# lashhw/rtcuda

Measured on AMD Instinct MI355X. Metric: Msamples/s at 1920x1080, bun_zipper.ply, higher is better.
Workload: dtype f32

## Files before the change

rtcuda_amd/csrc/rt_device.h:

```cpp
#ifndef RT_DEVICE_H
#define RT_DEVICE_H

#include <hip/hip_runtime.h>
#include <stdint.h>

#include "rt_pinned_math.h"

#define RT_DEV __device__ __forceinline__
#ifdef RT_ISA_MARKS
#define RT_MARK(name) __asm__ volatile("; RT_MARK " name)
#else
#define RT_MARK(name)
#endif

namespace rt {

constexpr float kInvPi = 0.31830988618379067153f;
constexpr float kTwoPi = 6.28318530717958647692f;
constexpr int kRrStart = 4;
constexpr float kRrThreshold = 1.f;
constexpr float kFltMax = 3.402823466e+38f;
constexpr float kFltEps = 1.192092896e-07f;

struct V3 {
    float x, y, z;
};
RT_DEV V3 mk(float x, float y, float z) { return V3{x, y, z}; }
RT_DEV V3 neg(V3 a) { return mk(-a.x, -a.y, -a.z); }
RT_DEV V3 add(V3 a, V3 b) { return mk(a.x + b.x, a.y + b.y, a.z + b.z); }
RT_DEV V3 sub(V3 a, V3 b) { return mk(a.x - b.x, a.y - b.y, a.z - b.z); }
RT_DEV V3 mul(V3 a, V3 b) { return mk(a.x * b.x, a.y * b.y, a.z * b.z); }
RT_DEV V3 scale(V3 a, float t) { return mk(a.x * t, a.y * t, a.z * t); }
RT_DEV V3 divf(V3 a, float t) {
    float inv_t = 1.f / t;
    return mk(a.x * inv_t, a.y * inv_t, a.z * inv_t);
}
RT_DEV float dot(V3 a, V3 b) { return a.x * b.x + a.y * b.y + a.z * b.z; }
RT_DEV V3 cross(V3 a, V3 b) {
    return mk(a.y * b.z - a.z * b.y, a.z * b.x - a.x * b.z, a.x * b.y - a.y * b.x);
}
RT_DEV float len2(V3 a) { return a.x * a.x + a.y * a.y + a.z * a.z; }
RT_DEV float len(V3 a) { return sqrtf(a.x * a.x + a.y * a.y + a.z * a.z); }
RT_DEV V3 unit(V3 a) {
    float inv_len = 1.f / len(a);
    return mk(a.x * inv_len, a.y * inv_len, a.z * inv_len);
}
RT_DEV float max3(V3 a) { return fmaxf(fmaxf(a.x, a.y), a.z); }
template <int STEPS = 1>
RT_DEV float rcp_exact_normal(float x) {
    float r = __builtin_amdgcn_rcpf(x);
#pragma unroll
    for (int k = 0; k < STEPS; k++) {
        const float e = fmaf(-x, r, 1.f);
        r = fmaf(e, r, r);
    }
    return r;
}
RT_DEV V3 reflect(V3 v, V3 n) { return sub(v, scale(n, 2.f * dot(v, n))); }
RT_DEV V3 refract4(V3 unit_v, V3 unit_n, float eta_ratio, float cos_theta) {
    V3 v_parallel = scale(add(unit_v, scale(unit_n, cos_theta)), eta_ratio);
    V3 v_perp = scale(unit_n, -sqrtf(1.f - len2(v_parallel)));
    return add(v_parallel, v_perp);
}

struct Rng {
    uint32_t d, v0, v1, v2, v3, v4;
};
RT_DEV uint32_t rng_next(Rng &s) {
    uint32_t t = s.v0 ^ (s.v0 >> 2);
    s.v0 = s.v1;
    s.v1 = s.v2;
    s.v2 = s.v3;
    s.v3 = s.v4;
    s.v4 = (s.v4 ^ (s.v4 << 4)) ^ (t ^ (t << 1));
    s.d += 362437u;
    return s.v4 + s.d;
}
RT_DEV Rng rng_sample_stream(uint32_t seed_lo, uint32_t seed_hi, unsigned long long key) {
    unsigned long long z = (((unsigned long long)seed_hi << 32) | seed_lo) + 0x9E3779B97F4A7C15ull * (key + 1ull);
    z = (z ^ (z >> 30)) * 0xBF58476D1CE4E5B9ull;
    z = (z ^ (z >> 27)) * 0x94D049BB133111EBull;
    z ^= z >> 31;
    const uint32_t s0 = (uint32_t)z ^ 0xaad26b49u, s1 = (uint32_t)(z >> 32) ^ 0xf7dcefddu;
    const uint32_t t0 = 1099087573u * s0, t1 = 2591861531u * s1;
    Rng r;
    r.d = 6615241u + t1 + t0;
    r.v0 = 123456789u + t0;
    r.v1 = 362436069u ^ t0;
    r.v2 = 521288629u + t1;
    r.v3 = 88675123u ^ t1;
    r.v4 = 5783321u + t0;
    return r;
}
RT_DEV float rng_to_uniform(uint32_t draw) { return (float)draw * 2.3283064e-10f + (2.3283064e-10f / 2.0f); }
RT_DEV float rng_uniform(Rng &s) { return rng_to_uniform(rng_next(s)); }

struct Tri {
    V3 p0, e1, e2, n;
};
RT_DEV Tri load_tri(const float4 *__restrict__ tris, int k) {
    const float4 *q = (const float4 *)((const char *)tris + __umul24((unsigned)k, 48u));
    float4 a = q[0];
    float4 b = q[1];
    float4 c = q[2];
    Tri t;
    t.p0 = mk(a.x, a.y, a.z);
    t.e1 = mk(a.w, b.x, b.y);
    t.e2 = mk(b.z, b.w, c.x);
    t.n = mk(c.y, c.z, c.w);
    return t;
}
RT_DEV bool tri_intersect(const Tri &tr, V3 o, V3 d, float tmax, float &t_out, float &u_out, float &v_out) {
    V3 c = sub(tr.p0, o);
    V3 r = cross(d, c);
    float inv_det = 1.f / dot(d, tr.n);
    float u = inv_det * dot(tr.e2, r);
    float v = inv_det * dot(tr.e1, r);
    float t = inv_det * dot(c, tr.n);
    t_out = t;
    u_out = u;
    v_out = v;
    return u >= 0.0f && v >= 0.0f && (u + v) <= 1.0f && 0 < t && t <= tmax;
}
RT_DEV V3 tri_point(const Tri &tr, float u, float v) { return add(sub(tr.p0, scale(tr.e1, u)), scale(tr.e2, v)); }
RT_DEV float tri_area(const Tri &tr) { return 0.5f * len(tr.n); }

RT_DEV V3 offset_ray_origin(V3 p, V3 n) {
    const float int_scale = 256.f;
    const float float_scale = 1.f / 65536.f;
    const float origin = 1.f / 32.f;
    int ox = (int)(int_scale * n.x);
    int oy = (int)(int_scale * n.y);
    int oz = (int)(int_scale * n.z);
    float px = __int_as_float(__float_as_int(p.x) + (p.x < 0 ? -ox : ox));
    float py = __int_as_float(__float_as_int(p.y) + (p.y < 0 ? -oy : oy));
    float pz = __int_as_float(__float_as_int(p.z) + (p.z < 0 ? -oz : oz));
    return mk(fabsf(p.x) < origin ? p.x + float_scale * n.x : px,
              fabsf(p.y) < origin ? p.y + float_scale * n.y : py,
              fabsf(p.z) < origin ? p.z + float_scale * n.z : pz);
}
RT_DEV float power_heuristic(float f_pdf, float g_pdf_float) {
    int g = (int)g_pdf_float;
    float f2 = f_pdf * f_pdf;
    return f2 / (f2 + (float)(g * g));
}
RT_DEV bool same_hemisphere(V3 wo, V3 wi, V3 n) { return dot(wo, n) * dot(wi, n) < 0.f; }
RT_DEV V3 uniform_sample_sphere(Rng &rs) {
    float z = 1 - 2 * rng_uniform(rs);
    float r = sqrtf(1 - z * z);
    float phi = kTwoPi * rng_uniform(rs);
    float x, y;
    rt_sincosf(phi, &y, &x);
    return mk(r * x, r * y, z);
}

struct Material {
    float ax, ay, az;
    float ior;
// ... 79 lines not shown
```

rtcuda_amd/csrc/rt_frame_kernels.inc:

```
#ifndef RT_CHUNK_RELEASE_WAIT
#define RT_CHUNK_RELEASE_WAIT 1
#endif

template <bool LDS_TABLES>
__global__ void __launch_bounds__(kBlock)
RT_K_ADVANCE(DScene sc, DPools p, RT_FRAME_SRC cam, AdvanceParams ap, float *__restrict__ fb, DCounters *__restrict__ ctr,
             DWaveRow *__restrict__ rows, unsigned int *__restrict__ lock_shades) {
    if (ap.lockstep >= 3 && lock_shades[ap.lockstep - 2] == 0u) return;
    __shared__ float s_tab[LDS_TABLES ? kTabDwordsMax : 1];
    const int i = blockIdx.x * blockDim.x + threadIdx.x;
    const bool in_range = i < ap.n;
    SlotState st;
    st.bounces = kDone;
    st.hit_info = -1;
    st.pixel = 0;
    st.gen = 0;
    st.rs = Rng{0, 0, 0, 0, 0, 0};
    st.beta = st.wo = st.isect_p = st.isect_n = mk(0, 0, 0);
    if (in_range) {
        st.bounces = p.bounces(i);
        st.hit_info = p.hit_info(i);
        st.pixel = p.pixel(i);
        st.gen = p.gen(i);
        st.rs = Rng{p.rd(i), p.r0(i), p.r1(i), p.r2(i), p.r3(i), p.r4(i)};
        st.beta = mk(p.br(i), p.bg(i), p.bb(i));
        st.wo = mk(p.dx(i), p.dy(i), p.dz(i));
        st.isect_p = mk(p.hpx(i), p.hpy(i), p.hpz(i));
        st.isect_n = mk(p.hnx(i), p.hny(i), p.hnz(i));
    }
    const float *tab = sc.tables;
    if (LDS_TABLES) {
        for (int k = threadIdx.x; k < sc.tab_dwords; k += kBlock) s_tab[k] = sc.tables[k];
        __syncthreads();
        tab = s_tab;
    }
    if (ap.lockstep && st.bounces == kParked) {
        st.bounces = ap.max_bounces;
        st.hit_info = -1;
    }
    const bool alive = st.bounces != kDone && st.bounces != kParked;
    AdvanceOut out;
    out.did_gen = out.did_shade = out.has_shadow = out.did_emit = out.new_ray = false;
    out.rr_draws = 0;
    if (alive) {
        const int gen_before = st.gen;
        advance_core<false>(sc, tab, cam, ap, ap.slot_lo + i, st, out, fb);
        if (out.new_ray) {
            p.ox(i) = out.ray_o.x;
            p.oy(i) = out.ray_o.y;
            p.oz(i) = out.ray_o.z;
            p.dx(i) = out.ray_d.x;
            p.dy(i) = out.ray_d.y;
            p.dz(i) = out.ray_d.z;
        }
        if (st.gen != gen_before) {
            p.gen(i) = st.gen;
            p.pixel(i) = st.pixel;
        }
        if (out.has_shadow) {
            p.sox(i) = out.s_o.x;
            p.soy(i) = out.s_o.y;
            p.soz(i) = out.s_o.z;
            p.sdx(i) = out.s_d.x;
            p.sdy(i) = out.s_d.y;
            p.sdz(i) = out.s_d.z;
            p.slr(i) = out.s_L.x;
            p.slg(i) = out.s_L.y;
            p.slb(i) = out.s_L.z;
            p.starget(i) = out.s_target;
            p.stmax(i) = out.s_tmax;
        }
        p.br(i) = st.beta.x;
        p.bg(i) = st.beta.y;
        p.bb(i) = st.beta.z;
        p.bounces(i) = st.bounces;
        p.rd(i) = st.rs.d;
        p.r0(i) = st.rs.v0;
        p.r1(i) = st.rs.v1;
        p.r2(i) = st.rs.v2;
        p.r3(i) = st.rs.v3;
        p.r4(i) = st.rs.v4;
    }
    if (in_range && !out.has_shadow) p.stmax(i) = -1.f;

    unsigned long long traced = wave_ballot(out.did_gen || out.did_shade);
    int rr_tot = out.rr_draws;
    if (wave_ballot(out.rr_draws != 0)) {
        for (int off = 32; off > 0; off >>= 1) rr_tot += __shfl_xor(rr_tot, off);
    } else {
        rr_tot = 0;
    }
    unsigned long long v[C_COUNT] = {(unsigned long long)wave_count((out.did_gen)),
                                     (unsigned long long)wave_count((out.did_shade)),
                                     (unsigned long long)__popcll(traced),
                                     (unsigned long long)wave_count((out.has_shadow)),
                                     (unsigned long long)wave_count((out.did_emit)),
                                     0ull,
                                     (unsigned long long)rr_tot,
                                     0ull};
    row_add(rows, v);
    if ((ap.round & ap.batch_mask) == ap.batch_mask && traced != 0 && lane_id() == 0) ctr->last_live_round = ap.round;
    if (ap.lockstep) {
        unsigned long long sm = wave_ballot(out.did_shade);
        if (sm != 0 && lane_id() == 0) atomicAdd(&lock_shades[ap.lockstep - 1], (unsigned)__popcll(sm));
    }
}

template <bool LDS_TABLES, bool WIDE, int MIN_WAVES, bool DRAW_CIDS = false, bool LITERAL = false, bool VERIFY = false>
__global__ void __launch_bounds__(kBlock, MIN_WAVES)
RT_K_PATHS(DScene sc, DPools p, RT_FRAME_SRC cam_arg, AdvanceParams ap_arg, float *__restrict__ fb, DWaveRow *__restrict__ rows,
           int stack_cap, int *overflow, int adv_batch, int debug_no_deposit, unsigned long long *prof, int top_n,
           int prio_period, int rot_wave, int rot_set, int gen_batch, int tri_follow, unsigned int *__restrict__ next_cid,
           unsigned long long *__restrict__ vstat) {
    constexpr bool SPLIT_GEN = MIN_WAVES != 2;
    asm volatile("s_nop 0\n\ts_nop 0");
    extern __shared__ int s_lds[];
    int *stack = s_lds + threadIdx.x;
    float *park = (float *)(s_lds + (stack_cap + 1) * kBlock) + threadIdx.x;
    int *over = overflow + (blockIdx.x * kBlock + threadIdx.x) % kOverStride;
    int *cold = s_lds + (stack_cap + 10) * kBlock + threadIdx.x;
    float *acc = (float *)(s_lds + (stack_cap + 23) * kBlock) + threadIdx.x;
    float *s_tab = (float *)(s_lds + (stack_cap + 26) * kBlock);
    const float *tab = sc.tables;
    const float4 *s_top = (const float4 *)(s_tab + (LDS_TABLES ? ((sc.tab_dwords + 3) & ~3) : 0));
    constexpr bool CHUNKS = RT_PATHS_CHUNKS && SPLIT_GEN && !DRAW_CIDS;
    __shared__ __attribute__((aligned(16))) unsigned s_task[CHUNKS ? 8 : 1];
    __shared__ unsigned s_sem[CHUNKS ? rtchunks::kSemWords : 1];
    const unsigned chunk_g0 = (CHUNKS && top_n > 0) ? (unsigned)top_n & ((1u << rtplan::kChunkHeadShift) - 1u) : 0u;
    const unsigned chunk_head0 = (CHUNKS && top_n > 0) ? (unsigned)top_n >> rtplan::kChunkHeadShift : 0u;
    if (CHUNKS) {
        for (unsigned k = threadIdx.x; k < rtchunks::kSemWords; k += kBlock) s_sem[k] = rtchunks::kSemWordInit;
        if (threadIdx.x == 0) {
            const rtchunks::Multiple m = rtchunks::multiple_of(chunk_g0 ? chunk_g0 : 1u);
            s_task[0] = 0u;
            s_task[1] = chunk_g0;
            s_task[2] = m.inv;
            s_task[3] = m.shift;
            s_task[4] = m.limit;
            s_task[5] = chunk_head0;
        }
    }
    const bool chunk_start = CHUNKS && chunk_g0 && chunk_head0 == 0u;
    if (MIN_WAVES != 2) top_n = 0;
    for (int k = threadIdx.x; k < top_n * 4; k += kBlock) ((float4 *)s_top)[k] = sc.nodes[k];
    if (LDS_TABLES) {
        for (int k = threadIdx.x; k < sc.tab_dwords; k += kBlock) s_tab[k] = sc.tables[k];
        tab = s_tab;
    }
    struct Uniforms {
        RT_FRAME_SRC cam;
        AdvanceParams ap;
    };
    static_assert(sizeof(Uniforms) % 4 == 0, "dword copy");
    Uniforms *s_uni = (Uniforms *)(s_top + 4 * (size_t)top_n);
    {
        Uniforms u;
        u.cam = cam_arg;
        u.ap = ap_arg;
        const int *srcw = (const int *)&u;
        for (int k = threadIdx.x; k < (int)(sizeof(Uniforms) / 4); k += kBlock) ((int *)s_uni)[k] = srcw[k];
    }
    __syncthreads();
    const RT_FRAME_SRC &cam = s_uni->cam;
    const AdvanceParams &ap = s_uni->ap;
    const int ap_n = ap_arg.n, ap_max_bounces = ap_arg.max_bounces, ap_fb_fixed = ap_arg.fb_fixed;
    constexpr bool draw_cids = DRAW_CIDS && SPLIT_GEN;
    int cid_next = 0, cid_end = 0;
    const int lanes_in_grid = (int)(gridDim.x * blockDim.x);
    auto slot_of = [&](int set, unsigned lane_in_wg) {
        return rtchunks::slot_of((unsigned)set, blockIdx.x * blockDim.x + lane_in_wg, (unsigned)lanes_in_grid, (unsigned)rot_wave, (unsigned)rot_set);
    };
    int slot_set = 0;
    int i = slot_of(0, threadIdx.x);
    int bounces = kDone, pixel = 0, gen = 0;
    Rng rs{0, 0, 0, 0, 0, 0};
    V3 beta = mk(0, 0, 0);
    auto load_slot = [&](int k) {
        bounces = p.bounces(k);
        pixel = p.pixel(k);
        gen = p.gen(k);
        rs = Rng{p.rd(k), p.r0(k), p.r1(k), p.r2(k), p.r3(k), p.r4(k)};
        beta = mk(p.br(k), p.bg(k), p.bb(k));
    };
    auto store_slot = [&](int k) {
        p.bounces(k) = bounces;
        p.pixel(k) = pixel;
        p.gen(k) = gen;
        p.hit_info(k) = -1;
        p.stmax(k) = -1.f;
        p.br(k) = beta.x;
        p.bg(k) = beta.y;
        p.bb(k) = beta.z;
        p.rd(k) = rs.d;
        p.r0(k) = rs.v0;
        p.r1(k) = rs.v1;
        p.r2(k) = rs.v2;
        p.r3(k) = rs.v3;
        p.r4(k) = rs.v4;
    };
    auto cold_save = [&]() {
        cold[0 * kBlock] = bounces;
        cold[1 * kBlock] = pixel;
        cold[2 * kBlock] = gen;
        cold[3 * kBlock] = (int)rs.d;
        cold[4 * kBlock] = (int)rs.v0;
        cold[5 * kBlock] = (int)rs.v1;
        cold[6 * kBlock] = (int)rs.v2;
        cold[7 * kBlock] = (int)rs.v3;
        cold[8 * kBlock] = (int)rs.v4;
        cold[9 * kBlock] = __float_as_int(beta.x);
        cold[10 * kBlock] = __float_as_int(beta.y);
        cold[11 * kBlock] = __float_as_int(beta.z);
    };
    auto cold_load = [&]() {
        bounces = cold[0 * kBlock];
        pixel = cold[1 * kBlock];
        gen = cold[2 * kBlock];
        rs = Rng{(uint32_t)cold[3 * kBlock], (uint32_t)cold[4 * kBlock], (uint32_t)cold[5 * kBlock],
                 (uint32_t)cold[6 * kBlock], (uint32_t)cold[7 * kBlock], (uint32_t)cold[8 * kBlock]};
        beta = mk(__int_as_float(cold[9 * kBlock]), __int_as_float(cold[10 * kBlock]), __int_as_float(cold[11 * kBlock]));
    };
    int phase = PH_IDLE;
// ... 23 lines not shown
    acc[0 * kBlock] = acc[1 * kBlock] = acc[2 * kBlock] = 0.f;
    if (chunk_start) {
        i = ap_n;
        phase = PH_GEN;
        cold[12 * kBlock] = -1;
    } else if (i < ap_n) {
        load_slot(i);
        phase = (bounces != kDone && bounces != kParked) ? (SPLIT_GEN ? PH_GEN : PH_ADV) : PH_IDLE;
        cold_save();
        cold[12 * kBlock] = -1;
    }
    unsigned long long n_gen = 0, n_shade = 0, n_traced = 0, n_shadow = 0, n_emit = 0, n_deposit = 0, n_rr = 0;
    unsigned n_bg_lane = 0;
#ifdef RT_TRACE_PROFILE
    unsigned long long pf[16] = {0, 0, 0, 0, 0, 0, 0, 0, 0, 0, 0, 0, 0, 0, 0, 0};
    unsigned long long pf_gen_cycles = 0, pf_fin_cycles = 0, pf_fin_lanes = 0, pf_fin_iters = 0;
    unsigned long long pf_handovers = 0, pf_handover_blocks = 0;
    const unsigned long long pf_t0 = __builtin_readcyclecounter();
    unsigned long long pf_last_work = 0;
#endif

    unsigned prio_tick = 0;
    const unsigned prio_rank = (4u * blockIdx.x) / gridDim.x;
    while (true) {
        RT_MARK("loop.head");
        if (prio_period && (prio_tick++ & ((1u << prio_period) - 1u)) == 0u) {
            unsigned lvl = ((prio_tick >> prio_period) + prio_rank) & 3u;
            lvl = max(lvl, prio_rank >> 1);
            switch (lvl) {
                case 0: __builtin_amdgcn_s_setprio(0); break;
                case 1: __builtin_amdgcn_s_setprio(1); break;
                case 2: __builtin_amdgcn_s_setprio(2); break;
                default: __builtin_amdgcn_s_setprio(3); break;
            }
        }
        bool trav = phase == PH_ANY || phase == PH_CLOSEST;
        bool want_node = trav && cur >= 0;
        bool want_tri = trav && ((cur != kEntryDone && cur < 0) || (kSpeculate && pend != kEntryDone));
        int n_adv = wave_count((phase == PH_ADV));
        const int n_genw = wave_count((phase == PH_GEN));
        int n_node = wave_count((want_node));
        int n_tri = wave_count((want_tri));
        if (n_adv + n_genw + n_node + n_tri == 0) break;
        auto retake = [&]() {
            trav = phase == PH_ANY || phase == PH_CLOSEST;
            want_node = trav && cur >= 0;
            want_tri = trav && ((cur != kEntryDone && cur < 0) || (kSpeculate && pend != kEntryDone));
            n_adv = wave_count((phase == PH_ADV));
            n_node = wave_count((want_node));
            n_tri = wave_count((want_tri));
        };
        const bool run_adv = n_adv > 0 && ((n_adv >= adv_batch && 2 * n_adv >= n_node && 2 * n_adv >= n_tri) || n_node + n_tri == 0);
        if (SPLIT_GEN && !run_adv && n_genw > 0 && (n_genw >= gen_batch || n_node + n_tri == 0)) {
            RT_MARK("gen.begin");
#ifdef RT_TRACE_PROFILE
            pf[12]++; pf[15] += n_genw;
            const unsigned long long pf_tg = __builtin_readcyclecounter();
#endif
            AdvanceOut out;
            out.did_gen = out.new_ray = false;
            out.ray_o = o;
            out.ray_d = d;
            bool hand_back = false;
            long long my_cid = -1;
            if (draw_cids) {
                const unsigned long long m = wave_ballot(phase == PH_GEN);
                const int need = (int)__popcll(m), rank = (int)prefix_popc(m);
                int served = 0;
                while (served < need) {
                    if (cid_next == cid_end) {
                        unsigned base = 0;
                        if (lane_id() == 0) base = atomicAdd(next_cid, (unsigned)kCidChunk);
                        static_assert(0x7ffff000u + (unsigned)kCidChunk < 0x7fffffffu, "cid_end must not overflow int");
                        cid_next = (int)min(__builtin_amdgcn_readfirstlane(base), 0x7ffff000u);
                        cid_end = cid_next + kCidChunk;
                    }
                    const int take = min(need - served, cid_end - cid_next);
                    if (phase == PH_GEN && rank >= served && rank < served + take) my_cid = cid_next + (rank - served);
                    cid_next += take;
                    served += take;
                }
            }
            const unsigned chunk_g = CHUNKS ? __builtin_amdgcn_readfirstlane(s_task[1]) : 0u;
            const bool chunk_was_gen = CHUNKS && phase == PH_GEN;
            const int chunk_acc_pixel = CHUNKS ? cold[1 * kBlock] : 0;
            if (CHUNKS && chunk_g) {
                const rtchunks::Multiple chunk_m{s_task[2], s_task[3], s_task[4]};
                const unsigned chunk_head = __builtin_amdgcn_readfirstlane(s_task[5]);
                bool need = phase == PH_GEN && i >= ap_n;
                const bool at_end = phase == PH_GEN && i < ap_n && slot_set >= (int)chunk_head &&
                                    rtchunks::chunk_ends((unsigned)cold[2 * kBlock], chunk_m, cold[0 * kBlock] == kChunkFresh);
                if (wave_ballot(need || at_end)) {
#ifdef RT_TRACE_PROFILE
                    bool pf_released = false;
#endif
                    if (at_end) {
                        cold_load();
                        const bool ends = gen == ap.last_gen || (long long)gen * kW + (ap.slot_lo + i) >= ap.cam_end;
                        if (!ends) {
                            bounces = ap_max_bounces;
                            store_slot(i);
                            const rtchunks::Owner own = rtchunks::owner_of((unsigned)i, (unsigned)lanes_in_grid, (unsigned)rot_wave, (unsigned)rot_set);
                            const unsigned idx = (own.set - chunk_head) * rtchunks::kLanes + (own.lane_in_grid & (rtchunks::kLanes - 1u));
#if RT_CHUNK_RELEASE_WAIT
                            __builtin_amdgcn_s_waitcnt(0x0f70);
#endif
                            const unsigned old = __hip_atomic_fetch_add(&s_sem[rtchunks::sem_word(idx) & (rtchunks::kSemWords - 1u)], rtchunks::sem_unit(idx),
                                                                        __ATOMIC_RELEASE, __HIP_MEMORY_SCOPE_WORKGROUP);
                            if (!rtchunks::runner_keeps(rtchunks::sem_value(old, idx))) {
                                i = ap_n;
                                need = true;
                            }
#ifdef RT_TRACE_PROFILE
                            pf_released = true;
#endif
                        }
                    }
#ifdef RT_TRACE_PROFILE
                    pf_handovers += wave_count(pf_released);
                    pf_handover_blocks += wave_ballot(pf_released) != 0 ? 1 : 0;
#endif
                    const unsigned chunk_sets = (unsigned)ap_n / (unsigned)lanes_in_grid - chunk_head;
                    const unsigned chunk_tasks = rtchunks::task_count(chunk_sets, (unsigned)ap.last_gen, (unsigned)chunk_g);
                    unsigned long long m;
                    while ((m = wave_ballot(need)) != 0ull) {
                        unsigned base = 0;
                        if (lane_id() == 0) base = atomicAdd(&s_task[0], (unsigned)__popcll(m));
                        const unsigned t = __builtin_amdgcn_readfirstlane(base) + prefix_popc(m);
                        if (need) {
                            if (t >= chunk_tasks) {
                                need = false;
                                phase = PH_IDLE;
                            } else {
                                const rtchunks::Entry e = rtchunks::task_entry(t, chunk_sets);
                                const int k = slot_of((int)(e.set + chunk_head), e.lane);
                                const unsigned idx = e.set * rtchunks::kLanes + e.lane;
                                const unsigned old = k < ap_n ? __hip_atomic_fetch_sub(&s_sem[rtchunks::sem_word(idx) & (rtchunks::kSemWords - 1u)], rtchunks::sem_unit(idx),
                                                                                       __ATOMIC_ACQUIRE, __HIP_MEMORY_SCOPE_WORKGROUP)
                                                              : rtchunks::kSemBias;
                                if (rtchunks::taker_runs(rtchunks::sem_value(old, idx))) {
                                    i = k;
                                    load_slot(i);
                                    cold_save();
                                    cold[0 * kBlock] = kChunkFresh;
                                    cold[12 * kBlock] = -1;
                                    need = false;
                                }
                            }
                        }
                    }
                }
            }
            if (CHUNKS) {
                __builtin_amdgcn_s_waitcnt(0x0f70);
                if (chunk_was_gen) acc_flush(acc, fb, ap_fb_fixed, chunk_acc_pixel);
            }
#if RT_PATHS_BG
            {
                static_assert((kW & (kW - 1)) == 0, "a slot's camera rays are counted with a shift");
                const bool was_gen = phase == PH_GEN;
                const int f_width = __builtin_amdgcn_readfirstlane(ap.width), f_dpx = __builtin_amdgcn_readfirstlane(ap.dpx);
                const int f_dpy = __builtin_amdgcn_readfirstlane(ap.dpy), f_last_gen = __builtin_amdgcn_readfirstlane(ap.last_gen);
                const int f_cam_end = __builtin_amdgcn_readfirstlane((int)ap.cam_end);
                const int f_slot_lo = __builtin_amdgcn_readfirstlane(ap.slot_lo);
                const int f_x0 = __builtin_amdgcn_readfirstlane(ap.bg_x0), f_y0 = __builtin_amdgcn_readfirstlane(ap.bg_y0);
                const unsigned f_w = (unsigned)__builtin_amdgcn_readfirstlane(ap.bg_w), f_h = (unsigned)__builtin_amdgcn_readfirstlane(ap.bg_h);
                const bool can_loop = !draw_cids && f_dpy >= 0;
                const rtchunks::Multiple bg_m{CHUNKS ? __builtin_amdgcn_readfirstlane(s_task[2]) : 1u, CHUNKS ? __builtin_amdgcn_readfirstlane(s_task[3]) : 0u,
                                              CHUNKS ? __builtin_amdgcn_readfirstlane(s_task[4]) : 0u};
                const bool dealt = CHUNKS && chunk_g && slot_set >= (int)__builtin_amdgcn_readfirstlane(s_task[5]);
                Rng g_rs{0, 0, 0, 0, 0, 0};
                int g_gen = 0, g_stop = 0, px = 0, py = 0;
                uint32_t draw_x = 0, draw_y = 0;
                bool looking = false, made = false;
                if (was_gen) {
                    g_gen = cold[2 * kBlock];
                    g_rs = Rng{(uint32_t)cold[3 * kBlock], (uint32_t)cold[4 * kBlock], (uint32_t)cold[5 * kBlock],
                               (uint32_t)cold[6 * kBlock], (uint32_t)cold[7 * kBlock], (uint32_t)cold[8 * kBlock]};
                    const int pxy = cold[12 * kBlock];
                    if (!CHUNKS) acc_flush(acc, fb, ap_fb_fixed, cold[1 * kBlock]);
                    const int slot = f_slot_lo + i;
                    if (draw_cids) g_stop = my_cid >= (long long)f_cam_end ? g_gen : 0x7fffffff;
                    else g_stop = min(f_last_gen, (f_cam_end - slot + (kW - 1)) >> __builtin_ctz((unsigned)kW));
                    looking = g_gen < g_stop;
                    px = pxy & 0xffff;
                    py = pxy >> 16;
                    if (looking && (pxy < 0 || !can_loop)) {
                        SlotState t;
                        t.gen = g_gen + 1;
                        int qx, qy;
                        gen_pixel(ap, slot, t, nullptr, my_cid, my_cid >= 0 ? my_cid : (long long)g_gen * kW + slot, qx, qy);
                        px = qx - f_dpx;
                        py = qy - f_dpy;
                        if (px < 0) {
                            px += f_width;
                            py--;
                        }
                    }
                }
                if (looking) {
                    bool bg;
                    do {
                        g_gen++;
                        px += f_dpx;
                        py += f_dpy;
                        if (px >= f_width) {
                            px -= f_width;
                            py++;
                        }
                        bg = (unsigned)(px - f_x0) >= f_w || (unsigned)(py - f_y0) >= f_h;
                        if (draw_cids) {
                            if (!bg) {
                                g_rs = rng_sample_stream(ap.seed_lo, ap.seed_hi, (unsigned long long)my_cid * (unsigned)ap.key_mul + (unsigned)ap.key_add);
                                draw_x = rng_next(g_rs);
                                draw_y = rng_next(g_rs);
                            }
                        } else {
                            draw_x = rng_next(g_rs);
                            draw_y = rng_next(g_rs);
                        }
                        n_bg_lane += bg ? 1u : 0u;
                    } while (bg && can_loop && g_gen < g_stop && !(dealt && rtchunks::chunk_ends((unsigned)g_gen, bg_m, false)));
                    made = !bg;
                }
                if (made) {
                    camera_get_ray(cam, (px + rng_to_uniform(draw_x)) / ap.width, (py + rng_to_uniform(draw_y)) / ap.height, out.ray_o, out.ray_d);
                    out.new_ray = true;
                    out.did_gen = true;
                }
                if (was_gen) {
                    int b = 0;
                    if (!made && g_gen >= g_stop) {
                        const long long cid = my_cid >= 0 ? my_cid : (long long)g_gen * kW + (f_slot_lo + i);
                        b = cid >= ap.cam_end ? kDone : kParked;
                        hand_back = true;
                    }
                    cold[0 * kBlock] = b;
                    cold[2 * kBlock] = g_gen;
                    cold[3 * kBlock] = (int)g_rs.d;
                    cold[4 * kBlock] = (int)g_rs.v0;
                    cold[5 * kBlock] = (int)g_rs.v1;
                    cold[6 * kBlock] = (int)g_rs.v2;
                    cold[7 * kBlock] = (int)g_rs.v3;
                    cold[8 * kBlock] = (int)g_rs.v4;
                    cold[12 * kBlock] = px | (py << 16);
                    if (made) {
                        cold[1 * kBlock] = py * f_width + px;
                        cold[9 * kBlock] = __float_as_int(1.f);
                        cold[10 * kBlock] = __float_as_int(1.f);
                        cold[11 * kBlock] = __float_as_int(1.f);
                    }
                }
            }
#else
            if (phase == PH_GEN) {
                SlotState st;
                st.gen = cold[2 * kBlock];
                st.rs = Rng{(uint32_t)cold[3 * kBlock], (uint32_t)cold[4 * kBlock], (uint32_t)cold[5 * kBlock],
                            (uint32_t)cold[6 * kBlock], (uint32_t)cold[7 * kBlock], (uint32_t)cold[8 * kBlock]};
                st.bounces = 0;
                st.pixel = 0;
                st.beta = mk(0, 0, 0);
                int pxy = cold[12 * kBlock];
                if (!CHUNKS) acc_flush(acc, fb, ap_fb_fixed, cold[1 * kBlock]);
                gen_core<true>(cam, ap, ap.slot_lo + i, st, out, &pxy, my_cid);
                cold[0 * kBlock] = st.bounces;
                cold[2 * kBlock] = st.gen;
                cold[3 * kBlock] = (int)st.rs.d;
                cold[4 * kBlock] = (int)st.rs.v0;
                cold[5 * kBlock] = (int)st.rs.v1;
                cold[6 * kBlock] = (int)st.rs.v2;
                cold[7 * kBlock] = (int)st.rs.v3;
                cold[8 * kBlock] = (int)st.rs.v4;
                if (out.new_ray) {
                    cold[1 * kBlock] = st.pixel;
                    cold[9 * kBlock] = __float_as_int(st.beta.x);
                    cold[10 * kBlock] = __float_as_int(st.beta.y);
                    cold[11 * kBlock] = __float_as_int(st.beta.z);
                    cold[12 * kBlock] = pxy;
                } else {
                    hand_back = true;
                }
            }
#endif
            const bool nr = out.new_ray;
            o = out.ray_o;
            d = out.ray_d;
            inv = inv_dir(d);
            phase = nr ? (int)PH_CLOSEST : phase;
            tmax = nr ? kFltMax : tmax;
            tri = nr ? -1 : tri;
            cur = nr ? 0 : cur;
            sp = nr ? 0 : sp;
            if (wave_ballot(hand_back)) {
                if (hand_back) {
                    if (draw_cids) {
                        phase = PH_IDLE;
                    } else if (CHUNKS && chunk_g && slot_set + 1 >= (int)s_task[5]) {
                        cold_load();
                        store_slot(i);
                        i = ap_n;
                        tri = -1;
                        slot_set = (int)s_task[5];
                    } else {
                        next_slot(PH_GEN);
                    }
                }
            }
            n_gen += wave_count((out.did_gen));
            n_traced += wave_count((out.new_ray));
#ifdef RT_TRACE_PROFILE
            pf_gen_cycles += __builtin_readcyclecounter() - pf_tg;
#endif
            retake();
            RT_MARK("gen.end");
        }
        if (run_adv) {
#ifdef RT_TRACE_PROFILE
            pf[0]++; pf[1] += n_adv;
            const unsigned long long pf_ta = __builtin_readcyclecounter();
#endif
            RT_MARK("adv.head");
            AdvanceOut out;
            out.did_gen = out.did_shade = out.has_shadow = out.did_emit = out.new_ray = false;
            out.rr_draws = 0;
            out.bg_skipped = 0;
            if (phase == PH_ADV) {
                cold_load();
                SlotState st;
                st.wo = d;
                st.hit_info = -1;
                st.isect_p = st.isect_n = mk(0, 0, 0);
                if (tri >= 0) {
                    Tri tr = load_tri(sc.tris, tri);
                    float4 sh = sc.tri_shade[(unsigned)tri];
                    RT_MARK("adv.verify");
                    if (VERIFY) {
                        bool bad = (__float_as_uint(hv) >> 31) != 0u;
                        if (bad) atomicAdd(&vstat[V_TIE], 1ull);
                        else bad = !ref_visible(sc, o, d, tr, tri, vstat);
                        if (bad) {
                            atomicAdd(&vstat[V_LITERAL], 1ull);
                            float tm = kFltMax;
                            tri = -1;
                            hu = hv = 0.f;
                            reference_walk<false>(sc, o, d, tm, tri, hu, hv, stack, over, stack_cap);
                            cold_load();
                            if (tri >= 0) {
                                tr = load_tri(sc.tris, tri);
                                sh = sc.tri_shade[(unsigned)tri];
                            }
                        }
                    }
                    RT_MARK("adv.hit_record");
                    if (!VERIFY || tri >= 0) {
                        st.isect_p = tri_point(tr, hu, hv);
                        st.isect_n = mk(sh.x, sh.y, sh.z);
                        st.hit_info = __float_as_int(sh.w);
                    }
                }
                st.bounces = bounces;
                st.pixel = pixel;
                st.gen = gen;
                st.rs = rs;
                st.beta = beta;
                advance_core<SPLIT_GEN, true, true, RT_PATHS_BG != 0>(sc, tab, cam, ap, ap.slot_lo + i, st, out, fb, acc);
                RT_MARK("adv.tail");
                bounces = st.bounces;
                pixel = st.pixel;
                gen = st.gen;
                rs = st.rs;
                beta = st.beta;
                if (out.has_shadow) {
                    park[0 * kBlock] = out.ray_o.x;
                    park[1 * kBlock] = out.ray_o.y;
                    park[2 * kBlock] = out.ray_o.z;
                    park[3 * kBlock] = out.ray_d.x;
                    park[4 * kBlock] = out.ray_d.y;
                    park[5 * kBlock] = out.ray_d.z;
                    park[6 * kBlock] = out.s_L.x;
                    park[7 * kBlock] = out.s_L.y;
                    park[8 * kBlock] = out.s_L.z;
                    o = out.s_o;
                    d = out.s_d;
                    phase = PH_ANY;
                    tmax = out.s_tmax;
// ... 252 lines not shown
```

rtcuda_amd/csrc/rt_host_check.cpp:

```cpp
#include <cfloat>
#include <cmath>
#include <cstdint>
#include <cstdio>
#include <cstring>
#include <cstdlib>
#include <vector>

#include "rt_background.h"
#include "rt_bvh.h"
#include "rt_denoise.h"
#include "rt_launch_plan.h"
#include "rt_ploc.h"
#include "rt_ref_tree.h"
#include "rt_slot_chunks.h"
#include "rt_stats_merge.h"
#include "rt_temporal.h"

namespace {
struct V3 { float x, y, z; };
inline V3 sub(V3 a, V3 b) { return {a.x - b.x, a.y - b.y, a.z - b.z}; }
inline float dot(V3 a, V3 b) { return a.x * b.x + a.y * b.y + a.z * b.z; }
inline V3 cross(V3 a, V3 b) { return {a.y * b.z - a.z * b.y, a.z * b.x - a.x * b.z, a.x * b.y - a.y * b.x}; }
struct Tri { V3 p0, e1, e2, n; };
inline bool tri_hit(const Tri &tr, V3 o, V3 d, float tmax, float &t) {
// ... 767 lines not shown
}
int rt_hostwalk_trace_verified(void *h, int mode, int n_rays, const float *o3, const float *d3, const float *tmax_in,
                               const int *excluded, int *out_i, float *out_t, long long *stats6) {
    const HostWalk &w = *(const HostWalk *)h;
    const rtbvh::Result &r = w.r;
    const std::vector<rtbvh::Pair> padded = w.wide ? padded_quads(r, n_rays, o3) : std::vector<rtbvh::Pair>();
    const std::vector<rtbvh::Pair> &rec = w.wide ? padded : r.pairs;
    const int stack_entries = w.wide ? r.stack_bound : r.pair_depth + 1;
    int failures = 0;
    long long own = 0, leafb = 0, ties = 0, negz = 0, lit = 0;
#pragma omp parallel for schedule(dynamic, 1024) reduction(+ : failures, own, leafb, ties, negz, lit)
    for (int i = 0; i < n_rays; i++) {
        V3 o{o3[3 * i], o3[3 * i + 1], o3[3 * i + 2]}, d{d3[3 * i], d3[3 * i + 1], d3[3 * i + 2]};
        const int excl = (mode == 1 && excluded[i] >= 0 && excluded[i] < w.n) ? w.inverse[excluded[i]] : -1;
        const RefSlab s = ref_slab(o, d);
        WalkResult res;
        negz += s.neg_zero ? 1 : 0;
        if (mode == 1) {
            res = walk_ray(rec, w.wide, w.tris, r.order, stack_entries, 1, o, d, tmax_in[i], excl, &w.ref);
            if (res.unseen_occluder) {
                lit++;
                const bool failed = res.failed;
                const long long of = res.own_fail, lf = res.leaf_fail;
                literal_walk(w, 1, o, d, tmax_in[i], excl, res);
                res.failed = failed; res.own_fail = of; res.leaf_fail = lf;
            }
        } else {
            res = walk_ray(rec, w.wide, w.tris, r.order, stack_entries, 0, o, d, tmax_in[i], -1);
            if (res.best >= 0) {
                const bool tie = res.tie_t == res.t;
                const bool seen = ref_visible(w.ref, s, w.tris[(size_t)res.best], r.order[(size_t)res.best], res);
                ties += tie ? 1 : 0;
                if (tie || !seen) {
                    lit++;
                    const bool failed = res.failed;
                    literal_walk(w, 0, o, d, tmax_in[i], -1, res);
                    res.failed = failed;
                }
            }
        }
        failures += res.failed ? 1 : 0;
        own += res.own_fail; leafb += res.leaf_fail;
        if (mode == 1) {
            out_i[i] = res.occluded ? 1 : 0;
        } else {
            out_i[i] = res.best >= 0 ? r.order[res.best] : -1;
            out_t[i] = res.t;
        }
    }
    if (stats6) { stats6[0] += n_rays; stats6[1] += own; stats6[2] += leafb; stats6[3] += ties; stats6[4] += negz; stats6[5] += lit; }
    return failures;
}
int rt_ref_tree_export(const float *tri9, int n, float *bounds6, int *count, int *link, int *prims, int *depth) {
    const rtref::Tree t = rtref::build(tri9, n);
    if (depth) *depth = t.depth;
    if (bounds6) {
        for (size_t i = 0; i < t.nodes.size(); i++) {
            memcpy(bounds6 + 6 * i, t.nodes[i].box.b, 24);
            count[i] = t.nodes[i].count;
            link[i] = t.nodes[i].link;
        }
        for (size_t i = 0; i < t.prims.size(); i++) prims[i] = t.prims[i];
    }
    return (int)t.nodes.size();
}
void rt_plan_paths_launch(int n, int cus, int wide, int n_nodes, int paths_cap, int lattice, int width, int spp, int64_t fixed_lds_bytes, int64_t *out10) {
    const rtplan::PathsLaunch p = rtplan::plan_paths_launch(n, cus, wide != 0, n_nodes, paths_cap, lattice != 0, width, spp, (size_t)fixed_lds_bytes);
    const int64_t v[10] = {p.blocks, p.few_blocks, (int64_t)p.lds_bytes, p.top_n, p.adv_batch, p.gen_batch, p.tri_follow, p.prio_rotate, p.rot_wave, p.rot_set};
    memcpy(out10, v, sizeof(v));
}
void rt_slot_chunk_tasks(int block, int sets, int lanes_in_grid, int rot_wave, int rot_set, uint32_t t0, int count, int32_t *slots, int32_t *levels) {
    for (int k = 0; k < count; k++) {
        const rtchunks::Entry e = rtchunks::task_entry(t0 + (uint32_t)k, (unsigned)sets);
        slots[k] = rtchunks::slot_of(e.set, (unsigned)block * rtchunks::kLanes + e.lane, (unsigned)lanes_in_grid, (unsigned)rot_wave, (unsigned)rot_set);
        levels[k] = (int32_t)e.level;
    }
}
int rt_slot_chunk_static_slot(int set, int lane_in_grid, int lanes_in_grid, int rot_wave, int rot_set) {
    return rtchunks::slot_of((unsigned)set, (unsigned)lane_in_grid, (unsigned)lanes_in_grid, (unsigned)rot_wave, (unsigned)rot_set);
}
uint32_t rt_slot_chunk_levels(uint32_t rays, uint32_t G) { return rtchunks::levels(rays, G); }
uint32_t rt_slot_chunk_task_count(uint32_t sets, uint32_t rays, uint32_t G) { return rtchunks::task_count(sets, rays, G); }
int rt_slot_chunk_ends(uint32_t gen, uint32_t G, int fresh) { return rtchunks::chunk_ends(gen, rtchunks::multiple_of(G), fresh != 0); }
int rt_slot_chunk_taker_runs(int old_sem) { return rtchunks::taker_runs(old_sem); }
int rt_slot_chunk_runner_keeps(int old_sem) { return rtchunks::runner_keeps(old_sem); }
int rt_plan_slot_chunk(int n, int cus, int chain) {
    return rtplan::slot_chunk_for(rtplan::plan_paths_launch(n, cus, true, 70000, 10, true, 1920, 256, 0), chain);
}
int rt_plan_slot_head(int n, int cus, int *sets_out) {
    const rtplan::PathsLaunch p = rtplan::plan_paths_launch(n, cus, true, 70000, 10, true, 1920, 256, 0);
    const int sets = n / (p.blocks * rtplan::kBlock);
    if (sets_out) *sets_out = sets;
    return rtplan::slot_head_for(p, sets);
}
int rt_plan_slot_chunk_if_resident(int chunk, int workgroups_per_cu) { return rtplan::slot_chunk_if_resident(chunk, workgroups_per_cu); }
void rt_slot_chunk_head_tasks(int block, int sets, int head, int lanes_in_grid, int rot_wave, int rot_set, uint32_t t0, int count, int32_t *slots, int32_t *levels, int32_t *idx) {
    for (int k = 0; k < count; k++) {
        const rtchunks::Entry e = rtchunks::task_entry(t0 + (uint32_t)k, (unsigned)(sets - head));
        slots[k] = rtchunks::slot_of(e.set + (unsigned)head, (unsigned)block * rtchunks::kLanes + e.lane, (unsigned)lanes_in_grid, (unsigned)rot_wave, (unsigned)rot_set);
        levels[k] = (int32_t)e.level;
        idx[k] = (int32_t)(e.set * rtchunks::kLanes + e.lane);
    }
}
void rt_slot_chunk_owner(int slot, int lanes_in_grid, int rot_wave, int rot_set, int32_t *out2) {
    const rtchunks::Owner o = rtchunks::owner_of((unsigned)slot, (unsigned)lanes_in_grid, (unsigned)rot_wave, (unsigned)rot_set);
    out2[0] = (int32_t)o.set;
    out2[1] = (int32_t)o.lane_in_grid;
}
uint32_t rt_slot_chunk_sem_word(uint32_t idx) { return rtchunks::sem_word(idx); }
uint32_t rt_slot_chunk_sem_unit(uint32_t idx) { return rtchunks::sem_unit(idx); }
int rt_slot_chunk_sem_value(uint32_t word, uint32_t idx) { return rtchunks::sem_value(word, idx); }
uint32_t rt_slot_chunk_sem_init() { return rtchunks::kSemWordInit; }
int rt_background_rect(const float cam12[12], int width, int height, const float lo[3], const float hi[3], int out4[4]) {
    if (!cam12 || !lo || !hi || !out4 || width <= 0 || height <= 0) return 1;
    const rtbg::Rect r = rtbg::background_rect(cam12, width, height, lo, hi);
    out4[0] = r.x0;
    out4[1] = r.y0;
    out4[2] = r.x1;
    out4[3] = r.y1;
    return 0;
}
int hc_denoise(const int64_t *sum_fixed, int num_samples, const int64_t *aov_fixed, int aov_samples, int width, int height, int passes,
               float sigma_color, float sigma_depth, int normal_power_log2, float *rgb_out) {
    if (!sum_fixed || !aov_fixed || !rgb_out || width < 1 || height < 1 || num_samples < 1 || aov_samples < 1) return 1;
    if (passes < 0 || passes > DN_MAX_PASSES || normal_power_log2 < 0 || normal_power_log2 > DN_MAX_NORMAL_POWER_LOG2) return 1;
    if (!(std::isfinite(sigma_color) && sigma_color > 0.f && std::isfinite(sigma_depth) && sigma_depth > 0.f)) return 1;
    const float sc2 = sigma_color * sigma_color, sd2 = sigma_depth * sigma_depth;
    const float kz = 1.f / sd2;
    float kc[DN_MAX_PASSES];
    for (int i = 0; i < passes; i++) {
        kc[i] = (float)(1 << (2 * i)) / sc2;
        if (!(std::isfinite(kc[i]) && kc[i] > 0.f)) return 1;
    }
    if (!(std::isfinite(kz) && kz > 0.f)) return 1;
    const size_t n = (size_t)width * (size_t)height;
    const float inv_spp = 1.f / (float)num_samples, inv_aov = 1.f / (float)aov_samples;
    std::vector<DnPixel> px(n);
    std::vector<float> uv(4 * n, 0.f);
    for (size_t p = 0; p < n; p++) {
        dn_prepare(sum_fixed + 3 * p, aov_fixed + DN_AOV_CHANNELS * p, inv_spp, inv_aov, &px[p]);
        for (int k = 0; k < 3; k++) uv[4 * p + k] = px[p].u[k];
    }
    dn_walk<false>(uv, px, width, height, passes, kc, kz, normal_power_log2);
    for (size_t p = 0; p < n; p++) dn_finish(&uv[4 * p], px[p].d, px[p].e, rgb_out + 3 * p);
    return 0;
}
void hc_expnegf(const float *x, float *y, int n) {
    for (int k = 0; k < n; k++) y[k] = rt_expnegf(x[k]);
}
int hc_denoise_dual(const int64_t *sum_a, int samples_a, const int64_t *sum_b, int samples_b, const int64_t *aov_fixed, int aov_samples,
                    int width, int height, int passes, float sigma_variance, float sigma_depth, int normal_power_log2, float *rgb_out,
                    float *var_out) {
    if (!sum_a || !sum_b || !aov_fixed || !rgb_out || width < 1 || height < 1 || samples_a < 1 || samples_b < 1 || aov_samples < 1) return 1;
    if ((long long)samples_a + samples_b > 0x7fffffffll) return 1;
    if (passes < 0 || passes > DN_MAX_PASSES || normal_power_log2 < 0 || normal_power_log2 > DN_MAX_NORMAL_POWER_LOG2) return 1;
    if (!(std::isfinite(sigma_variance) && sigma_variance > 0.f && std::isfinite(sigma_depth) && sigma_depth > 0.f)) return 1;
    const float ks = sigma_variance * sigma_variance, sd2 = sigma_depth * sigma_depth;
    const float kz = 1.f / sd2;
    if (!(std::isfinite(ks) && ks > 0.f && std::isfinite(kz) && kz > 0.f)) return 1;
    const int ns = samples_a + samples_b;
    const float kv = (float)((double)samples_a * (double)samples_b / ((double)ns * (double)ns));
    const float inv_a = 1.f / (float)samples_a, inv_b = 1.f / (float)samples_b, inv_n = 1.f / (float)ns, inv_aov = 1.f / (float)aov_samples;
    const size_t n = (size_t)width * (size_t)height;
    std::vector<DnPixel> px(n);
    std::vector<float> uv(4 * n);
    for (size_t p = 0; p < n; p++) {
// ... 110 lines not shown
```

rtcuda_amd/csrc/rt_slot_chunks.h:

```cpp
#pragma once

#if defined(__HIPCC__)
#define RT_CHUNKS_FN __host__ __device__ inline
#else
#define RT_CHUNKS_FN inline
#endif

namespace rtchunks {
constexpr unsigned kLanes = 256;

RT_CHUNKS_FN unsigned levels(unsigned rays, unsigned G) { return (rays + G - 1u) / G; }
RT_CHUNKS_FN unsigned task_count(unsigned sets, unsigned rays, unsigned G) { return sets * kLanes * levels(rays, G); }

struct Entry {
    unsigned set, lane, level;
};
RT_CHUNKS_FN Entry task_entry(unsigned t, unsigned sets) {
    const unsigned S = sets * kLanes, idx = t % S;
    return Entry{idx / kLanes, idx % kLanes, t / S};
}

RT_CHUNKS_FN int slot_of(unsigned set, unsigned lane_in_grid, unsigned lanes_in_grid, unsigned rot_wave, unsigned rot_set) {
    const unsigned wave_in_grid = lane_in_grid >> 6, lane_in_wave = lane_in_grid & 63u;
    const unsigned b = (wave_in_grid + (wave_in_grid & 3u) * rot_wave + set * rot_set) & ((lanes_in_grid >> 6) - 1u);
    return (int)(set * lanes_in_grid + b * 64u + lane_in_wave);
}

RT_CHUNKS_FN bool taker_runs(int old_sem) { return old_sem >= 1; }
RT_CHUNKS_FN bool runner_keeps(int old_sem) { return old_sem < 0; }

constexpr unsigned kSemBias = 0x4000u, kSemBanked = kSemBias + 1u;
constexpr unsigned kSemWordInit = kSemBanked | (kSemBanked << 16);
constexpr unsigned kDealtSetsMax = 4;
constexpr unsigned kSemWords = kDealtSetsMax * kLanes / 2u;
static_assert(kSemBias > 2046u && kSemBias + 1u < 0x10000u, "a field must hold [bias - 2046, bias + 1]");
RT_CHUNKS_FN unsigned sem_word(unsigned idx) { return idx >> 1; }
RT_CHUNKS_FN unsigned sem_unit(unsigned idx) { return 1u << (16u * (idx & 1u)); }
RT_CHUNKS_FN int sem_value(unsigned word, unsigned idx) { return (int)((word >> (16u * (idx & 1u))) & 0xffffu) - (int)kSemBias; }

struct Owner {
    unsigned set, lane_in_grid;
};
RT_CHUNKS_FN Owner owner_of(unsigned slot, unsigned lanes_in_grid, unsigned rot_wave, unsigned rot_set) {
    const unsigned mask = (lanes_in_grid >> 6) - 1u;
    const unsigned set = slot >> (31u - (unsigned)__builtin_clz(lanes_in_grid)), b = (slot >> 6) & mask;
    const unsigned low = (b - set * rot_set) & 3u;
    const unsigned wave = (b - low * rot_wave - set * rot_set) & mask;
    return Owner{set, wave * 64u + (slot & 63u)};
}

struct Multiple {
    unsigned inv, shift, limit;
};
RT_CHUNKS_FN Multiple multiple_of(unsigned G) {
    unsigned shift = 0;
    while (((G >> shift) & 1u) == 0u) shift++;
    const unsigned odd = G >> shift;
    unsigned inv = odd;
    for (int k = 0; k < 5; k++) inv *= 2u - odd * inv;
    return Multiple{inv, shift, 0xffffffffu / G};
}
RT_CHUNKS_FN bool is_multiple(unsigned gen, const Multiple &m) {
    const unsigned q = gen * m.inv;
    return ((q >> m.shift) | (m.shift ? q << (32u - m.shift) : 0u)) <= m.limit;
}
RT_CHUNKS_FN bool chunk_ends(unsigned gen, const Multiple &m, bool fresh) { return !fresh && is_multiple(gen, m); }
}
```

Before: 5215.

## Precompute background-skip loop limit and batch RNG Weyl updates in gen loop

Rewrites the per-lane background pixel-skip loop so that its exit bound is computed once up front with a reciprocal-multiply next-multiple formula, replacing the per-iteration chunk_ends divisibility test. The xorshift state step is split from the Weyl counter, which is now advanced once after the loop by a 24-bit multiply. Wrap handling and the background test become branchless, and the chunk parameters are read from LDS once with vector loads. A host-side exhaustive checker is added to confirm run_limit matches the old loop semantics. The risk is a subtle mismatch in RNG draws or loop bounds, and the extra scalar registers the new values need.

```diff
diff --git a/rtcuda_amd/csrc/rt_device.h b/rtcuda_amd/csrc/rt_device.h
--- a/rtcuda_amd/csrc/rt_device.h
+++ b/rtcuda_amd/csrc/rt_device.h
@@ -66,14 +66,18 @@
 struct Rng {
     uint32_t d, v0, v1, v2, v3, v4;
 };
-RT_DEV uint32_t rng_next(Rng &s) {
+constexpr uint32_t kRngWeyl = 362437u;
+RT_DEV void rng_step(Rng &s) {
     uint32_t t = s.v0 ^ (s.v0 >> 2);
     s.v0 = s.v1;
     s.v1 = s.v2;
     s.v2 = s.v3;
     s.v3 = s.v4;
     s.v4 = (s.v4 ^ (s.v4 << 4)) ^ (t ^ (t << 1));
-    s.d += 362437u;
+}
+RT_DEV uint32_t rng_next(Rng &s) {
+    rng_step(s);
+    s.d += kRngWeyl;
     return s.v4 + s.d;
 }
 RT_DEV Rng rng_sample_stream(uint32_t seed_lo, uint32_t seed_hi, unsigned long long key) {
diff --git a/rtcuda_amd/csrc/rt_frame_kernels.inc b/rtcuda_amd/csrc/rt_frame_kernels.inc
--- a/rtcuda_amd/csrc/rt_frame_kernels.inc
+++ b/rtcuda_amd/csrc/rt_frame_kernels.inc
@@ -1,5 +1,11 @@
 #ifndef RT_CHUNK_RELEASE_WAIT
 #define RT_CHUNK_RELEASE_WAIT 1
+#endif
+#undef RT_GEN_CHUNK_HEAD
+#if RT_PATHS_BG
+#define RT_GEN_CHUNK_HEAD (int)tk_head
+#else
+#define RT_GEN_CHUNK_HEAD (int)s_task[5]
 #endif
 
 template <bool LDS_TABLES>
@@ -138,6 +144,9 @@
             s_task[3] = m.shift;
             s_task[4] = m.limit;
             s_task[5] = chunk_head0;
+#if RT_PATHS_BG
+            s_task[6] = rtchunks::next_multiple_mul(chunk_g0 ? chunk_g0 : 1u);
+#endif
         }
     }
     const bool chunk_start = CHUNKS && chunk_g0 && chunk_head0 == 0u;
@@ -327,11 +336,28 @@
                 }
             }
             const unsigned chunk_g = CHUNKS ? __builtin_amdgcn_readfirstlane(s_task[1]) : 0u;
+#if RT_PATHS_BG
+            unsigned tk_inv = 1u, tk_shift = 0u, tk_limit = 0u, tk_head = 0u, tk_mul = 0u;
+            if (CHUNKS) {
+                const uint2 lo = *(const uint2 *)&s_task[2];
+                const uint4 hi = *(const uint4 *)&s_task[4];
+                tk_inv = __builtin_amdgcn_readfirstlane(lo.x);
+                tk_shift = __builtin_amdgcn_readfirstlane(lo.y);
+                tk_limit = __builtin_amdgcn_readfirstlane(hi.x);
+                tk_head = __builtin_amdgcn_readfirstlane(hi.y);
+                tk_mul = __builtin_amdgcn_readfirstlane(hi.z);
+            }
+#endif
             const bool chunk_was_gen = CHUNKS && phase == PH_GEN;
             const int chunk_acc_pixel = CHUNKS ? cold[1 * kBlock] : 0;
             if (CHUNKS && chunk_g) {
+#if RT_PATHS_BG
+                const rtchunks::Multiple chunk_m{tk_inv, tk_shift, tk_limit};
+                const unsigned chunk_head = tk_head;
+#else
                 const rtchunks::Multiple chunk_m{s_task[2], s_task[3], s_task[4]};
                 const unsigned chunk_head = __builtin_amdgcn_readfirstlane(s_task[5]);
+#endif
                 bool need = phase == PH_GEN && i >= ap_n;
                 const bool at_end = phase == PH_GEN && i < ap_n && slot_set >= (int)chunk_head &&
                                     rtchunks::chunk_ends((unsigned)cold[2 * kBlock], chunk_m, cold[0 * kBlock] == kChunkFresh);
@@ -411,11 +437,9 @@
                 const int f_x0 = __builtin_amdgcn_readfirstlane(ap.bg_x0), f_y0 = __builtin_amdgcn_readfirstlane(ap.bg_y0);
                 const unsigned f_w = (unsigned)__builtin_amdgcn_readfirstlane(ap.bg_w), f_h = (unsigned)__builtin_amdgcn_readfirstlane(ap.bg_h);
                 const bool can_loop = !draw_cids && f_dpy >= 0;
-                const rtchunks::Multiple bg_m{CHUNKS ? __builtin_amdgcn_readfirstlane(s_task[2]) : 1u, CHUNKS ? __builtin_amdgcn_readfirstlane(s_task[3]) : 0u,
-                                              CHUNKS ? __builtin_amdgcn_readfirstlane(s_task[4]) : 0u};
-                const bool dealt = CHUNKS && chunk_g && slot_set >= (int)__builtin_amdgcn_readfirstlane(s_task[5]);
+                const bool dealt = CHUNKS && chunk_g && slot_set >= (int)tk_head;
                 Rng g_rs{0, 0, 0, 0, 0, 0};
-                int g_gen = 0, g_stop = 0, px = 0, py = 0;
+                int g_gen = 0, g_stop = 0, g_limit = 0, px = 0, py = 0;
                 uint32_t draw_x = 0, draw_y = 0;
                 bool looking = false, made = false;
                 if (was_gen) {
@@ -428,13 +452,15 @@
                     if (draw_cids) g_stop = my_cid >= (long long)f_cam_end ? g_gen : 0x7fffffff;
                     else g_stop = min(f_last_gen, (f_cam_end - slot + (kW - 1)) >> __builtin_ctz((unsigned)kW));
                     looking = g_gen < g_stop;
+                    g_limit = (int)rtchunks::run_limit((unsigned)g_gen, (unsigned)g_stop, dealt, can_loop, chunk_g, tk_mul);
                     px = pxy & 0xffff;
                     py = pxy >> 16;
                     if (looking && (pxy < 0 || !can_loop)) {
                         SlotState t;
                         t.gen = g_gen + 1;
                         int qx, qy;
-                        gen_pixel(ap, slot, t, nullptr, my_cid, my_cid >= 0 ? my_cid : (long long)g_gen * kW + slot, qx, qy);
+                        const unsigned cid32 = draw_cids ? (unsigned)my_cid : (unsigned)g_gen * (unsigned)kW + (unsigned)slot;
+                        gen_pixel(ap, slot, t, nullptr, (long long)cid32, (long long)cid32, qx, qy);
                         px = qx - f_dpx;
                         py = qy - f_dpy;
                         if (px < 0) {
@@ -445,28 +471,37 @@
                 }
                 if (looking) {
                     bool bg;
+                    const int g_entry = g_gen;
+                    RT_MARK("gen.loop.begin");
                     do {
                         g_gen++;
                         px += f_dpx;
-                        py += f_dpy;
-                        if (px >= f_width) {
-                            px -= f_width;
-                            py++;
+                        const bool wrap = px >= f_width;
+                        px = (int)min((unsigned)px, (unsigned)(px - f_width));
+                        py += f_dpy + (wrap ? 1 : 0);
+                        bg = ((unsigned)(px - f_x0) >= f_w) | ((unsigned)(py - f_y0) >= f_h);
+                        if (!draw_cids) {
+                            rng_step(g_rs);
+                            rng_step(g_rs);
                         }
-                        bg = (unsigned)(px - f_x0) >= f_w || (unsigned)(py - f_y0) >= f_h;
-                        if (draw_cids) {
-                            if (!bg) {
-                                g_rs = rng_sample_stream(ap.seed_lo, ap.seed_hi, (unsigned long long)my_cid * (unsigned)ap.key_mul + (unsigned)ap.key_add);
-                                draw_x = rng_next(g_rs);
-                                draw_y = rng_next(g_rs);
-                            }
-                        } else {
+                    } while (!draw_cids && (bg & (g_gen < g_limit)));
+                    RT_MARK("gen.loop.end");
+                    __asm__ volatile("" : "+v"(px), "+v"(py));
+                    made = !(((unsigned)(px - f_x0) >= f_w) | ((unsigned)(py - f_y0) >= f_h));
+                    const uint32_t turns = (uint32_t)(g_gen - g_entry);
+                    n_bg_lane += turns - (made ? 1u : 0u);
+                    if (draw_cids) {
+                        if (made) {
+                            g_rs = rng_sample_stream(ap.seed_lo, ap.seed_hi, (unsigned long long)my_cid * (unsigned)ap.key_mul + (unsigned)ap.key_add);
                             draw_x = rng_next(g_rs);
                             draw_y = rng_next(g_rs);
                         }
-                        n_bg_lane += bg ? 1u : 0u;
-                    } while (bg && can_loop && g_gen < g_stop && !(dealt && rtchunks::chunk_ends((unsigned)g_gen, bg_m, false)));
-                    made = !bg;
+                    } else {
+                        static_assert(2u * kRngWeyl < (1u << 24), "a 24-bit multiply");
+                        g_rs.d += __umul24(turns, 2u * kRngWeyl);
+                        draw_x = g_rs.v3 + (g_rs.d - kRngWeyl);
+                        draw_y = g_rs.v4 + g_rs.d;
+                    }
                 }
                 if (made) {
                     camera_get_ray(cam, (px + rng_to_uniform(draw_x)) / ap.width, (py + rng_to_uniform(draw_y)) / ap.height, out.ray_o, out.ray_d);
@@ -541,12 +576,12 @@
                 if (hand_back) {
                     if (draw_cids) {
                         phase = PH_IDLE;
-                    } else if (CHUNKS && chunk_g && slot_set + 1 >= (int)s_task[5]) {
+                    } else if (CHUNKS && chunk_g && slot_set + 1 >= RT_GEN_CHUNK_HEAD) {
                         cold_load();
                         store_slot(i);
                         i = ap_n;
                         tri = -1;
-                        slot_set = (int)s_task[5];
+                        slot_set = RT_GEN_CHUNK_HEAD;
                     } else {
                         next_slot(PH_GEN);
                     }
diff --git a/rtcuda_amd/csrc/rt_host_check.cpp b/rtcuda_amd/csrc/rt_host_check.cpp
--- a/rtcuda_amd/csrc/rt_host_check.cpp
+++ b/rtcuda_amd/csrc/rt_host_check.cpp
@@ -873,6 +873,48 @@
 uint32_t rt_slot_chunk_levels(uint32_t rays, uint32_t G) { return rtchunks::levels(rays, G); }
 uint32_t rt_slot_chunk_task_count(uint32_t sets, uint32_t rays, uint32_t G) { return rtchunks::task_count(sets, rays, G); }
 int rt_slot_chunk_ends(uint32_t gen, uint32_t G, int fresh) { return rtchunks::chunk_ends(gen, rtchunks::multiple_of(G), fresh != 0); }
+uint32_t rt_slot_chunk_next_multiple(uint32_t gen, uint32_t G) { return rtchunks::next_multiple(gen, G, rtchunks::next_multiple_mul(G)); }
+uint32_t rt_slot_chunk_run_limit(uint32_t gen, uint32_t g_stop, int dealt, int can_loop, uint32_t G) {
+    return rtchunks::run_limit(gen, g_stop, dealt != 0, can_loop != 0, G, rtchunks::next_multiple_mul(G));
+}
+void rt_slot_chunk_run_limit_check(uint32_t g_lo, uint32_t g_hi, int64_t *out4) {
+    int64_t runs = 0, bad = 0, first_G = -1, first_gen = -1;
+#pragma omp parallel for schedule(dynamic, 8) reduction(+ : runs, bad)
+    for (int64_t G = g_lo; G <= (int64_t)g_hi; G++) {
+        const rtchunks::Multiple m = rtchunks::multiple_of((uint32_t)G);
+        const uint32_t mul = rtchunks::next_multiple_mul((uint32_t)G);
+        uint32_t next = 0;
+        for (uint32_t gen = 0; gen <= 2047u; gen++) {
+            if (next <= gen) next += (uint32_t)G;
+            const uint32_t stops[5] = {gen + 1u, next - 1u, next, next + 1u, 2047u};
+            for (uint32_t g_stop : stops) {
+                if (!(gen < g_stop)) continue;
+                for (int dealt = 0; dealt < 2; dealt++)
+                    for (int can_loop = 0; can_loop < 2; can_loop++) {
+                        uint32_t a = gen, b = gen;
+                        do a++;
+                        while (can_loop && a < g_stop && !(dealt && rtchunks::chunk_ends(a, m, false)));
+                        const uint32_t limit = rtchunks::run_limit(gen, g_stop, dealt != 0, can_loop != 0, (uint32_t)G, mul);
+                        do b++;
+                        while (b < limit);
+                        runs++;
+                        if (a != b) {
+                            bad++;
+#pragma omp critical
+                            if (first_G < 0 || G < first_G) {
+                                first_G = G;
+                                first_gen = gen;
+                            }
+                        }
+                    }
+            }
+        }
+    }
+    out4[0] = runs;
+    out4[1] = bad;
+    out4[2] = first_G;
+    out4[3] = first_gen;
+}
 int rt_slot_chunk_taker_runs(int old_sem) { return rtchunks::taker_runs(old_sem); }
 int rt_slot_chunk_runner_keeps(int old_sem) { return rtchunks::runner_keeps(old_sem); }
 int rt_plan_slot_chunk(int n, int cus, int chain) {
diff --git a/rtcuda_amd/csrc/rt_slot_chunks.h b/rtcuda_amd/csrc/rt_slot_chunks.h
--- a/rtcuda_amd/csrc/rt_slot_chunks.h
+++ b/rtcuda_amd/csrc/rt_slot_chunks.h
@@ -65,4 +65,18 @@
     return ((q >> m.shift) | (m.shift ? q << (32u - m.shift) : 0u)) <= m.limit;
 }
 RT_CHUNKS_FN bool chunk_ends(unsigned gen, const Multiple &m, bool fresh) { return !fresh && is_multiple(gen, m); }
+
+RT_CHUNKS_FN unsigned next_multiple_mul(unsigned G) { return (0x80000000u + G - 1u) / G; }
+RT_CHUNKS_FN unsigned next_multiple(unsigned gen, unsigned G, unsigned mul) {
+    return ((unsigned)(((unsigned long long)(2u * gen + 1u) * mul) >> 32) + 1u) * G;
 }
+RT_CHUNKS_FN unsigned run_limit(unsigned gen, unsigned g_stop, bool dealt, bool can_loop, unsigned G, unsigned mul) {
+    unsigned limit = g_stop;
+    if (dealt) {
+        const unsigned e = next_multiple(gen, G, mul);
+        limit = e < limit ? e : limit;
+    }
+    if (!can_loop) limit = gen + 1u < limit ? gen + 1u : limit;
+    return limit;
+}
+}
```

After: 5465, median of 6. 1.05x the previous value.
